# moss-lab/ScanFold

Measured on AMD Instinct MI355X. Metric: windows/sec (W=120, step=1, 100 shuffles), higher is better.
Workload: dtype int32 (int16 LDS storage) energies; f64 partition function

## Files before the change

scanfold_amd/csrc/sf_mfe_fast.hip.h:

```cpp
#pragma once
#include <type_traits>
#include "sf_energy.h"
#include "sf_pk16.h"

#define SF_FAST_NR 34
#ifndef SF_FAST_TINY_D0
#define SF_FAST_TINY_D0 10
#endif
#define SF_FAST_CHUNK_D0 36
#ifndef SF_FAST_UNPACK
#define SF_FAST_UNPACK 1
#endif
#ifndef SF_UNP_PB
#define SF_UNP_PB 4
#endif
#define SF_HELP_MERGE_MAXW 118
#define SF_DML_HELPER_BIAS_256 26
#define SF_DML_HELPER_BIAS_W200 50
#define SF_DML_HELPER_BIAS(ng, wt) ((ng) == 256 ? ((wt) == 200 ? SF_DML_HELPER_BIAS_W200 : SF_DML_HELPER_BIAS_256) : 100000)
#define SF_HELP_NB_128 4
#define SF_HELP_NB_128G 8
#define SF_HELP_NB_256 6
#define SF_INF16 30000
#define SF_FAST_THRESH 10000
// ... 219 lines not shown
      b[k] = pbl[BP ? k * S : (NB - 1 - k) * (S - 1)];
    }
    SF_SPLIT_REDUCE()
  } else {
#pragma unroll
    for (int k = 0; k < NB; k++) {
      const int t = k < NB - 1 ? sfd_min(k, len - 1) : len - 1;
      a[k] = pa[t * sa];
      b[k] = pb[t * sb];
    }
    SF_SPLIT_REDUCE()
  }
#undef SF_SPLIT_REDUCE
}

__device__ __forceinline__ void sf_fast_publish_bn(int16_t *w, const int i0, const uint32_t bn) {
  w[0] = (int16_t)sf_lo(bn);
  if (i0 > 0) w[-1] = (int16_t)sf_hi(bn);
}

#ifdef SF_EMUL
#define SF_GATHER16(F, field, idx) ((int)(F)->field[idx])
#else
__device__ __forceinline__ int sf_gather16_at(const void *base, unsigned off) {
  asm("" : "+v"(off));
  return *(const int16_t *)((const char *)base + (size_t)off);
}
#define SF_GATHER16(F, field, idx) \
  (FOLD ? sf_gather16_at((F), (unsigned)offsetof(SfFastParams, field) + ((unsigned)(idx) << 1)) : (int)(F)->field[idx])
#endif

#ifdef SF_EMUL
static thread_local const char *sf_emul_bn_base = nullptr, *sf_emul_ci_base = nullptr;
static inline void sf_emul_check_bn_row(const char *row_ptr, long lane_bytes, long row_bytes, bool fold) {
  if (!sf_emul_bn_base) return;
  const long row = (row_ptr - sf_emul_bn_base - lane_bytes) / row_bytes;
  if (row < 0 || row > (fold ? SF_FAST_NR - 1 : SF_FAST_NR)) {
    fprintf(stderr, "sf_mfe_fast (emulation): bulge / 1xn row %ld outside the ring and its mirror row\n", row);
    abort();
  }
}
static inline void sf_emul_check_ci_row(const int16_t *row_ptr, long lane_entries, long row_entries, bool fold) {
  if (!sf_emul_ci_base) return;
  const long row = ((const char *)row_ptr - sf_emul_ci_base - 2 * lane_entries) / (2 * row_entries);
  if (row < 0 || row > (fold ? SF_FAST_NR - 1 : SF_FAST_NR)) {
    fprintf(stderr, "sf_mfe_fast (emulation): generic-loop row %ld outside the ring and its mirror row\n", row);
    abort();
  }
}
#endif

enum { SF_SEC_P1 = 1, SF_SEC_HELP = 2, SF_SEC_DML = 4, SF_SEC_FIN = 8, SF_SEC_C0 = 16, SF_SEC_ALL = 31, SF_SEC_PRE = 32,
       SF_SEC_POST = 64 };
struct SfHU {
  short v[27];
};
struct SfPub {
  uint32_t a;
  uint32_t b;
  int tau;
  int type;
};
template <bool G, int WT, int SEC, bool CH = false, bool FOLD = false, int UCAP = SFD_MAXLOOP, int TBLK = 1, bool MGH = false,
          bool UNP = false>
__device__ __forceinline__ void sf_fast_cell(const SfFastCtx &X, const int d, const int i, const bool valid,
                                             const int slot2, const int slotd, uint32_t (&HP)[14], SfHU &HU, int &ovf,
                                             const bool final_fml, const int fnb, int &fpart, int &dec, int &eh, int &e0,
                                             int &dprev, SfPub &pub, const int dml_lo = SFD_TURN + 1,
                                             const int dml_hi = 1 << 20) {
  const SfFastParams *const Fc = FOLD ? X.F : sf_const_base(X.F);
  const int16_t *const ubase = G ? X.uNIN : (CH ? Fc->uniG[sfd_max(sfd_min(d - 2 - (SFD_TURN + 1), 30), 0)] : Fc->uni);
  const int16_t *const uNIN = ubase, *const uIL = ubase + 32, *const uBN = ubase + 64;
#define CBAT(x) X.BN[2 * (x)]
#define C1NAT(x) X.BN[2 * ((x) - 1) + 1]
#define HGET(x) (((x)&1) ? ((int)HP[(x) >> 1] >> 16) : (int)(int16_t)(HP[(x) >> 1] & 0xffffu))
#define HSET(x, v)                                                                                       \
  HP[(x) >> 1] = ((x)&1) ? ((HP[(x) >> 1] & 0x0000ffffu) | ((uint32_t)(v) << 16))                         \
                         : ((HP[(x) >> 1] & 0xffff0000u) | ((uint32_t)(v)&0xffffu))
  const int W = WT ? WT : X.W, RW = W - 4;
// ... 15 lines not shown
    const int tau_in = tr > 2 ? X.TAU : 0;
    int stem, ext;
    if (i > 1 && j < W) { stem = X.tM[SF_TIDX(type, sp1, sq1)]; ext = X.tE[SF_TIDX(type, sp1, sq1)]; }
    else if (i > 1) stem = ext = X.tD5[type * 5 + sp1];
    else if (j < W) stem = ext = X.tD3[type * 5 + sq1];
    else stem = ext = 0;
    pub.a = sf_pk(X.tI[SF_TIDX(tr, sq1, sp1)], X.t1n[SF_TIDX(tr, sq1, sp1)]);
    pub.b = sf_pk(stem + tau_in + X.MLintern, ext + tau_in);
    pub.tau = tau_in;
  }
#define FBASE(dd) (FOLD ? ((dd) <= (W + 3) / 2 ? ((dd)-4) * (W - 3) : (W - 1 - (dd)) * (W - 3) + (dd)-3) \
                        : (((dd)-4) * W - ((dd) * ((dd)-1) / 2 - 6) + (((dd)-4 + (W & 1)) >> 1)))
#define FLEN(dd) (W - (dd) + ((W - (dd)) & 1))
#define ROW(u) ((slot2 - (u) < 0 ? slot2 - (u) + SF_FAST_NR : slot2 - (u)) * RW)
  constexpr bool TBL = !G && TBLK != 0;
  const SfFastRows *const Rc = TBL ? sf_const_base(X.R) : X.R;
  const int32_t *const rci_o = Rc->ci_odd[slot2], *const rci_e = Rc->ci_even[slot2];
  const int32_t *const rbn_o = Rc->bn_odd[slot2], *const rbn_e = Rc->bn_even[slot2];
#define ROWB_CI(u) (TBL ? (((u)&1) ? rci_o[(u) >> 1] : rci_e[(u) >> 1]) : 2 * ROW(u))
#define ROWB_BN(u) (TBL ? (((u)&1) ? rbn_o[(u) >> 1] : rbn_e[(u) >> 1]) : 4 * ROW(u))
#define CIROW(u) ((const int16_t *)((const char *)X.CI + ROWB_CI(u)))

  if (SEC & SF_SEC_P1) {
  if (UNP) {
    static_assert(!UNP || (!G && !CH && !FOLD), "the unpacked recurrence exists for the all-sizes code of the narrow kernel only");
    const int32_t *const nin = Fc->NIN;
    short r30a = 0, r30b = 0;
    {
      const int16_t *row = CIROW(30) + i0;
      r30a = row[3]; r30b = row[29];
    }
    constexpr int PB = SF_UNP_PB;
#pragma unroll
    for (int pb = 12; pb >= 1; pb -= PB) {
      short a3[PB], au[PB], b3[PB], bu[PB];
#pragma unroll
      for (int k = 0; k < PB; k++) {
        if (pb - k >= 1) {
          const int u = 2 * (pb - k) + 4;
          const int16_t *rb = CIROW(u + 1) + i0, *ra = rb + RW;
#ifdef SF_EMUL
          sf_emul_check_ci_row(ra, i0, RW, FOLD); sf_emul_check_ci_row(rb, i0, RW, FOLD);
#endif
          a3[k] = ra[3]; au[k] = ra[u - 1];
          b3[k] = rb[3]; bu[k] = rb[u];
        }
      }
      if (pb == 12) {
        const short e = (short)(sf_opaque16(sfd_min16(r30a, r30b)) + (short)nin[26]);
        HU.v[26] = sf_opaque16(sfd_min16(e, HU.v[24]));
      }
#pragma unroll
      for (int k = 0; k < PB; k++) {
        if (pb - k >= 1) {
          const int x = 2 * (pb - k);
          const short ea = (short)(sf_opaque16(sfd_min16(a3[k], au[k])) + (short)nin[x]);
          const short eb = (short)(sf_opaque16(sfd_min16(b3[k], bu[k])) + (short)nin[x + 1]);
          HU.v[x + 1] = sf_opaque16(sfd_min16(eb, HU.v[x - 1]));
          HU.v[x] = sf_opaque16(sfd_min16(ea, HU.v[x - 2]));
        }
      }
    }
    {
      const int16_t *row = CIROW(5) + i0;
      HU.v[1] = (short)(sfd_min16((short)row[3], (short)row[4]) + (short)nin[1]);
      HU.v[0] = (short)((short)(CIROW(4) + i0)[3] + (short)nin[0]);
    }
  } else {
  if (G) {
#pragma unroll
    for (int u = 30; u >= 6; --u) {
      if (u <= UCAP && u <= umax) {
        const int16_t *row = X.CI + ROW(u) + i0;
        const int e = sfd_min(row[3], row[u - 1]) + SF_UNI(uNIN, u - 4);
        HSET(u - 4, sfd_min(e, HGET(u - 6)));
      }
    }
  } else {
    if (!CH || um >= 30) {
// ... 71 lines not shown
      }
      if (!G || (UCAP >= 3 && umax >= 3)) {
        const int16_t *row = BNROWB(ROWB_BN(3));
        const unsigned ta = RP[S[i + 2] * 8 + S[j - 3]];
        eh = sfd_min(eh, row[2 * 2] + SF_GATHER16(Fc, int21a, (((tq + ta) * 5u + si1) * 5u + S[j - 2]) * 5u + sj1));
        const unsigned tb = RP[S[i + 3] * 8 + S[j - 2]];
        eh = sfd_min(eh, row[2 * 3] + SF_GATHER16(Fc, int21b, (((tb * 8u + type) * 5u + sj1) * 5u + si1) * 5u + S[i + 2]));
      }
      if (!G || (UCAP >= 4 && umax >= 4)) {
        const unsigned t2r = RP[S[i + 3] * 8 + S[j - 3]];
        eh = sfd_min(eh, BNROWB(ROWB_BN(4))[2 * 3] +
                             SF_GATHER16(Fc, int22T, ((((tq + t2r) * 5u + si1) * 5u + S[i + 2]) * 5u + S[j - 2]) * 5u + sj1));
      }
      if (!G || (UCAP >= 5 && umax >= 5)) {
        const int16_t *row = BNROWB(ROWB_BN(5));
        const int m23 = X.t23[SF_TIDX(type, si1, sj1)] + Fc->L23;
        const int ta = RP[S[i + 3] * 8 + S[j - 4]];
        eh = sfd_min(eh, row[2 * 3] + m23 + X.t23in[SF_TIDX(ta, S[j - 3], S[i + 2])]);
        const int tb = RP[S[i + 4] * 8 + S[j - 3]];
        eh = sfd_min(eh, row[2 * 4] + m23 + X.t23in[SF_TIDX(tb, S[j - 2], S[i + 3])]);
      }
      int gb = SF_FAST_BIG, g1 = SF_FAST_BIG;
      if (G) {
#pragma unroll
        for (int u = 2; u <= 30; ++u) {
          if (u <= UCAP && u <= umax) {
            const int rw = ROW(u) + i0;
            gb = sfd_min(gb, sfd_min(CBAT(rw + 1), CBAT(rw + 1 + u)) + SF_UNI(uBN, 2 * u));
            if (u >= 4) g1 = sfd_min(g1, sfd_min(C1NAT(rw + 2), C1NAT(rw + u)) + SF_UNI(uBN, 2 * u + 1));
          }
        }
      } else {
        constexpr bool STAGED = (WT == 120);
        uint32_t acc = sf_pk(32767, 32767), accb = acc;
        constexpr int SF_HELP_NB = FOLD ? SF_HELP_NB_256 : (TBLK == 2 ? SF_HELP_NB_128G : SF_HELP_NB_128);
#pragma unroll
        for (int ub = 2; ub <= 30; ub += SF_HELP_NB) {
          if (CH && ub > um) continue;
          uint32_t w0[SF_HELP_NB], w2[SF_HELP_NB], w3[SF_HELP_NB], wt[SF_HELP_NB], t[SF_HELP_NB];
#pragma unroll
          for (int k = 0; k < SF_HELP_NB; k++) {
            const int u = ub + k;
            if (u <= 30) {
              const int16_t *tp = (FOLD || MGH || u == 30) ? BNROWB(ROWB_BN(u)) : BNROWB(ROWB_BN(u | 1)) + ((u & 1) ? 0 : 2 * RW);
#ifdef SF_EMUL
              sf_emul_check_bn_row((const char *)tp, 4 * i0, 4 * RW, FOLD);
#endif
              w0[k] = sf_ldw(tp + 2 * 1);
              w2[k] = sf_ldw(tp + 2 * (u - 1)); w3[k] = sf_ldw(tp + 2 * (u + 1));
              wt[k] = sf_ldw(uBN + 2 * u);
            }
          }
          if (STAGED) {
#pragma unroll
            for (int k = 0; k < SF_HELP_NB; k++) {
              const int u = ub + k;
              if (u <= 30) {
                const uint32_t x = w0[k];
                const uint32_t y = (w3[k] & 0xffffu) | (w2[k] & 0xffff0000u);
                t[k] = sf_pkmin(x, y);
              }
            }
            SF_VALU_FENCE();
#pragma unroll
            for (int k = 0; k < SF_HELP_NB; k++)
              if (ub + k <= 30) t[k] = sf_pkadd(t[k], wt[k]);
            SF_VALU_FENCE();
#pragma unroll
            for (int k = 0; k + 1 < SF_HELP_NB; k += 2)
              if (ub + k + 1 <= 30) t[k] = sf_pkmin(t[k], t[k + 1]);
            SF_VALU_FENCE();
#pragma unroll
            for (int k = 0; k < SF_HELP_NB; k += 2)
              if (ub + k <= 30) { if (k & 2) accb = sf_pkmin(accb, t[k]); else acc = sf_pkmin(acc, t[k]); }
          } else {
#pragma unroll
            for (int k = 0; k < SF_HELP_NB; k++) {
              const int u = ub + k;
              if (u <= 30) {
                const uint32_t x = w0[k];
                const uint32_t y = (w3[k] & 0xffffu) | (w2[k] & 0xffff0000u);
                acc = sf_pkmin(acc, sf_pkadd(sf_pkmin(x, y), wt[k]));
              }
            }
          }
        }
        acc = sf_pkmin(acc, accb);
        gb = sf_lo(acc); g1 = sf_hi(acc);
      }
      eh = sfd_min(eh, gb + tau_out);
      eh = sfd_min(eh, g1 + X.t1n[SF_TIDX(type, si1, sj1)]);
    }
  }

// ... 68 lines not shown
          const int n = size == 4 ? X.D->P.n_tetra : (size == 6 ? X.D->P.n_hexa : X.D->P.n_tri);
          const uint32_t key = sfd_loop_key(S, i, size + 2);
          for (int k0 = ((n + 7) & ~7) - 8; k0 >= 0; k0 -= 8) {
#pragma unroll
            for (int k = 7; k >= 0; --k) e = keys[k0 + k] == key ? (int)en[k0 + k] : e;
          }
        }
      } else e = X.D->hp_init[d - 1] + X.tH[SF_TIDX(type, si1, sj1)];
      if (!G || umax >= 0) {
        int gg = SF_FAST_BIG;
        if (UNP) {
          const int32_t *const il = Fc->IL;
          short g0 = (short)(HU.v[2] + (short)il[6]), g1 = (short)(HU.v[3] + (short)il[7]);
#pragma unroll
          for (int x = 4; x <= 26; x += 2) {
            g0 = sfd_min16(g0, sf_opaque16((short)(HU.v[x] + (short)il[x + 4])));
            if (x + 1 <= 26) g1 = sfd_min16(g1, sf_opaque16((short)(HU.v[x + 1] + (short)il[x + 5])));
          }
          gg = sfd_min16(g0, g1);
        } else if (G) {
#pragma unroll
          for (int u = 6; u <= 30; ++u)
            if (u <= UCAP && u <= umax) gg = sfd_min(gg, HGET(u - 4) + SF_UNI(uIL, u));
        } else {
          uint32_t ggp = sf_pk(32767, 32767);
#pragma unroll
          for (int pp = 1; pp <= 13; pp++)
            if (!CH || um >= 2 * pp + 4) ggp = sf_pkmin(ggp, sf_pkadd(HP[pp], sf_ldw(uIL + 2 * pp + 4)));
          gg = sfd_min(sf_lo(ggp), sf_hi(ggp));
        }
        e = sfd_min(e, gg + X.tI[SF_TIDX(type, si1, sj1)]);
      }
// ... 33 lines not shown
    const uint32_t bn = sf_pk(c + tau_in, c + X.t1n[SF_TIDX(tr, sq1, sp1)]);
    sf_fast_publish_bn(X.BN + 2 * rbd, i0, bn);
    if (X.bn_dup && slotd == 0) sf_fast_publish_bn(X.BN + 2 * (SF_FAST_NR * RW + i0), i0, bn);
    int stem, ext;
    if (i > 1 && j < W) { stem = X.tM[SF_TIDX(type, sp1, sq1)]; ext = X.tE[SF_TIDX(type, sp1, sq1)]; }
    else if (i > 1) stem = ext = X.tD5[type * 5 + sp1];
    else if (j < W) stem = ext = X.tD3[type * 5 + sq1];
    else stem = ext = 0;
    f = c + stem + tau_in + X.MLintern;
    cx = sfd_min(c + ext + tau_in, SF_INF16);
  } else {
    X.CI[rbd] = SF_INF16; sf_fast_publish_bn(X.BN + 2 * rbd, i0, sf_pk(SF_INF16, SF_INF16));
    if (!FOLD && slotd == 0) X.CI[SF_FAST_NR * RW + i0] = SF_INF16;
    if (X.bn_dup && slotd == 0) sf_fast_publish_bn(X.BN + 2 * (SF_FAST_NR * RW + i0), i0, sf_pk(SF_INF16, SF_INF16));
  }
  X.cg[SF_CGIDX(i, j)] = (int16_t)cx;
  if (final_fml && d > SFD_TURN + 1) f = sfd_min(f, fnb);
  if ((SEC & SF_SEC_DML) && (SEC & SF_SEC_FIN)) multiloop_split();
  f = sfd_min(f, dec);
  dprev = dec > SF_FAST_THRESH ? SF_INF16 : dec;
  fpart = f;
  if (final_fml && f < SF_FAST_OVF) ovf = 1;
  X.fML[FBASE(d) + i0] = (int16_t)(f > SF_FAST_THRESH ? SF_INF16 : f);
#undef ROW
#undef ROWB_CI
#undef ROWB_BN
#undef CIROW
#undef BNROWB
}

// ... 359 lines not shown
                                                int32_t *__restrict__ out, int *__restrict__ ovf_cnt,
                                                int *__restrict__ ovf_list) {
  if (lane == 0) {
    out[seq] = T.f3n;
    if (over || T.f3n < SF_FAST_OVF) {
      const int k = atomicAdd(ovf_cnt, 1);
      ovf_list[k] = seq;
    }
  }
}


enum SfStep {
  SF_STEP_SIZED,
  SF_STEP_GUARDED,
  SF_STEP_UNSPLIT,
  SF_STEP_SPLIT,
  SF_STEP_SPLIT16,
  SF_STEP_SPLIT8,
  SF_STEP_NARROW,
};
template <SfStep K>
using SfStepTag = std::integral_constant<SfStep, K>;
enum SfRole {
  SF_ROLE_ALL,
  SF_ROLE_MAIN_EVEN,
  SF_ROLE_MAIN_ODD,
  SF_ROLE_HELP_EVEN,
  SF_ROLE_HELP_ODD,
};
// ... 21 lines not shown
  const int W = WT ? WT : Wrt;
  SF_DYN_SMEM(smem);
  const SfFastLayout Lo = sf_fast_layout(W, HC);
  SfFastCtx X;
  char *const hcC = (char *)(smem + Lo.off_hc);
  uint8_t *const hcP = (uint8_t *)hcC + (W + 2), *const hcE = hcP + (W + 2);
  int16_t *const scS = (int16_t *)(smem + Lo.off_hc + (((3 * (W + 2)) + 1) & ~1));
  X.hc.c = (HC && cons_rows) ? hcC : nullptr; X.hc.partner = hcP; X.hc.encl = hcE;
  X.sc = (HC && sc_rows) ? scS : nullptr;
  X.fML = (int16_t *)smem;
  X.CI = (int16_t *)(smem + Lo.off_ci);
  X.C1N = nullptr; X.CB = nullptr;
  X.BN = (int16_t *)(smem + Lo.off_c1n);
#ifdef SF_EMUL
  sf_emul_bn_base = (const char *)X.BN; sf_emul_ci_base = (const char *)X.CI;
#endif
  X.DMLr = nullptr;
  int16_t *tab = (int16_t *)(smem + Lo.off_tab);
  X.t23 = tab; X.tI = tab + 175 - 25; X.t1n = tab + 325 - 25; X.tM = tab + 475 - 25; X.tH = tab + 625 - 25;
  X.tE = tab + 775 - 25; X.cg_ext = 1;
  X.tStack = tab + 925; X.tD5 = tab + 989; X.tD3 = tab + 1029;
  uint8_t *tPair = (uint8_t *)(tab + 1069);
  X.tPair = tPair;
  uint8_t *tRPair = (uint8_t *)(tab + SF_FAST_TAB_OLD);
  int16_t *t23in = tab + SF_FAST_TAB_OLD + 32;
  X.tRPair = tRPair; X.t23in = t23in;
  int32_t *flag = (int32_t *)(smem + Lo.off_flag);
  uint8_t *S = (uint8_t *)(smem + Lo.off_S);
  X.S = S;
  X.D = D; X.F = F; X.R = Rows; X.W = W; X.fold = FOLD; X.maxd = D->max_pair_dist;
  constexpr bool MERGE = MG && (NG == 128);
  constexpr bool UNPK = SF_FAST_UNPACK && (NG == 128);
  constexpr bool LGLOOPS = MG && (NG == 128);
  constexpr bool ROLE_LOOPS = (NG == 128);
  constexpr int TBLK = WT > 0 ? 1 : (NG == 128 ? (MG ? 2 : 1) : 0);
  X.bn_dup = (NG == 128);
  uint8_t *const cell_list = (MG && W >= SF_HELP_MERGE_MAXW) ? (uint8_t *)((int16_t *)(smem + Lo.off_tab) + 1069 + 32 + 1)
                                                            : (uint8_t *)(smem + Lo.off_list);
  X.TAU = D->P.TerminalAU; X.MLbase = D->P.MLbase; X.MLclosing = D->P.MLclosing; X.MLintern = D->P.MLintern[1];
  int32_t *f5s = (int32_t *)(smem + Lo.off_ci);
  int16_t *tExt = (int16_t *)(smem + Lo.off_ci + (((W + 1) * 4 + 3) & ~3));

  const int tid = threadIdx.x;
  X.cg = cg_all + (size_t)sf_fast_scratch_slot(blockIdx.x, gridDim.x) * SF_CG_ENTRIES(W);
  for (int x = tid; x < 175; x += NT) {
    tab[x] = F->mm23[x];
    if (x < 150) {
// ... 32 lines not shown
  const int defer_need = n_split_steps > 0 ? (W - SFD_TURN - 1 + n_split_steps - 1) / n_split_steps : 0;
  const int defer_rows = sfd_min(defer_need, DROWS);
  const bool defer_on = n_split_steps >= 8 && defer_need <= 4;
  SfTrail<NQ> T;
#pragma unroll
  for (int q = 0; q < NQ; q++) T.F[q] = 0;
  T.f3n = 0; T.row = 0;

  int *const next_slot = (int *)(smem + Lo.off_next);
  int seq = blockIdx.x;
  while (seq < n) {
    const uint8_t *src = seqs + (size_t)seq * W;
    constexpr bool PINF = true;
    int tidf = tid;
    if (PINF) SF_PIN(tidf);
    __syncthreads();
    if (PZ) {
      for (int x = tid; x < Lo.off_tab / 2; x += NT) ((int16_t *)smem)[x] = sf_poison16(poison, x);
      if (HC) for (int x = tid; x < (Lo.total - Lo.off_hc) / 2; x += NT) ((int16_t *)(smem + Lo.off_hc))[x] = sf_poison16(poison, x);
      __syncthreads();
    }
    for (int x = tidf; x < W; x += NT) S[x + 1] = sf_encode_nt(src[x]);
    if (MG && W >= SF_HELP_MERGE_MAXW) for (int x = tidf; x < 128; x += NT) ((int16_t *)(smem + Lo.off_tab) + 1069 + 32 + 1)[x] = F->uni[x];
    for (int x = tidf; x < (Lo.off_tab - Lo.off_ci) / 4; x += NT) ((uint32_t *)X.CI)[x] = sf_pk(SF_INF16, SF_INF16);
    int fetched = 0;
    if (tid == 0) {
      S[0] = 0; S[W + 1] = 0; flag[0] = 0;
      fetched = (int)gridDim.x + atomicAdd(work_ctr, 1);
    }
    __syncthreads();
    if (HC) {
      if (cons_rows)
        for (int x = tid; x < W; x += NT) hcC[x + 1] = cons_rows[(size_t)seq * W + x];
      if (sc_rows)
        for (int x = tid; x < W; x += NT) scS[x + 1] = (int16_t)sfd_max(sfd_min(sc_rows[(size_t)seq * W + x], 30000), -30000);
      __syncthreads();
      if (cons_rows && tid == 0) flag[0] = sf_hc_parse8(W, hcC, hcP, hcE) ? 2 : 0;
      __syncthreads();
      if (cons_rows && flag[0] == 2) {
// ... 20 lines not shown
    int slot2 = (SFD_TURN + 1 + grp - 2) % SF_FAST_NR, slotd = (SFD_TURN + 1 + grp) % SF_FAST_NR;
    auto build_list = [&](const int dd0) {
      const int lane = tid & 63;
      const int d1 = dd0 + 1;
      const int iH = ((v - 64) & (NG - 1)) - (dd0 >> 1);
      const bool vA = (dd0 < W) && (iH >= 1) && (iH + dd0 <= W), vB = (d1 < W) && (iH >= 1) && (iH + d1 <= W);
      const int tA = (vA && dd0 <= X.maxd) ? X.tPair[S[iH] * 8 + S[iH + dd0]] : 0;
      const int tB = (vB && d1 <= X.maxd) ? X.tPair[S[iH] * 8 + S[iH + d1]] : 0;
      const unsigned long long mA = __ballot(tA != 0), mB = __ballot(tB != 0);
      const int cA = __popcll(mA);
      uint8_t *list = cell_list + (((dd0 >> 1) & 1) << 7);
      const unsigned long long below = (1ull << lane) - 1ull;
      if (tA) list[__popcll(mA & below)] = (uint8_t)iH;
      if (tB) list[cA + __popcll(mB & below)] = (uint8_t)(iH | 128);
      if (lane == 0) list[127] = (uint8_t)(cA + __popcll(mB));
    };
    SfHU HU;
    const int grp_wave = grp;
    const bool sweeper_wave = sweeper;
    auto step = [&](const int d0, auto kind_tag, auto role_tag) {
      constexpr SfStep KIND = decltype(kind_tag)::value;
      constexpr SfRole ROLE = decltype(role_tag)::value;
      constexpr bool ROLES = ROLE != SF_ROLE_ALL;
      static_assert(!ROLES || (NG == 128 && KIND >= SF_STEP_SPLIT && KIND <= SF_STEP_SPLIT8), "roles: the narrow kernel's split steps");
      const int grp = ROLES ? (int)(ROLE == SF_ROLE_MAIN_ODD || ROLE == SF_ROLE_HELP_ODD) : grp_wave;
      const bool hwave = ROLES ? ROLE >= SF_ROLE_HELP_EVEN : tg >= 64;
      const bool sweeper = ROLES ? ROLE == SF_ROLE_HELP_ODD : sweeper_wave;
      constexpr int LGC = KIND == SF_STEP_SPLIT16 ? 4 : (KIND == SF_STEP_SPLIT8 ? 3 : (KIND == SF_STEP_SPLIT && LGLOOPS ? 5 : 0));
      constexpr bool DO_G = KIND == SF_STEP_SIZED, DO_CH = KIND == SF_STEP_GUARDED;
      const int d = d0 + grp;
      if (!ROLES && d0 == SFD_TURN + 1 + 2 && tid == 0) *next_slot = fetched;
      if (!ROLES && d0 == SFD_TURN + 1 + 4) next_seq = SF_WAVE_UNIFORM(*next_slot);
      constexpr bool split = KIND >= SF_STEP_SPLIT;
      constexpr bool narrow = KIND == SF_STEP_NARROW;
      if (NARROW && d0 == narrow_d0) {
        uint32_t *const xa = (uint32_t *)X.BN;
        const int RWc = W - 4;
        if (tg >= 96 && tg < 160) {
#pragma unroll
          for (int k = 0; k < 14; k++) xa[(grp * 16 + k) * RWc + 100 + (tg - 96)] = H[k];
          xa[(grp * 16 + 14) * RWc + 100 + (tg - 96)] = (uint32_t)dprev;
          xa[(grp * 16 + 15) * RWc + 100 + (tg - 96)] = (uint32_t)fnb;
        }
        __syncthreads();
        if (tg >= 64 && tg < 128) {
// ... 19 lines not shown
      int dec = SF_FAST_BIG, eh = SF_FAST_BIG, e0 = SF_FAST_BIG;
      SfPub pub;
      pub.a = pub.b = 0; pub.tau = 0; pub.type = 0;
      int dc[DROWS][NQ];
      const bool sweep_now = defer_on && sweeper && split && T.row > 0;
      const int sweep_rows = sweep_now ? sfd_max(sfd_min(defer_rows, T.row - (W - d0)), 0) : 0;
      if (sweep_now) {
#pragma unroll
        for (int k = 0; k < DROWS; k++)
          if (k < sweep_rows) sf_trail_load<NQ>(X.cg, W, tid & 63, T.row - k, dc[k]);
      }
      if (__ballot(valid)) {
        if (DO_G && d0 < 8) sf_fast_cell<true, WT, SF_SEC_ALL, false, FOLD, 1>(X, d, i, valid, slot2, slotd, H, HU, ovf, grp == 0, fnb, fpart, dec, eh, e0, dprev, pub);
        else if (DO_G && d0 < SF_FAST_TINY_D0) sf_fast_cell<true, WT, SF_SEC_ALL, false, FOLD, 5>(X, d, i, valid, slot2, slotd, H, HU, ovf, grp == 0, fnb, fpart, dec, eh, e0, dprev, pub);
        else if (DO_CH && d0 < SF_FAST_CHUNK_D0) sf_fast_cell<false, WT, SF_SEC_ALL, true, FOLD, SFD_MAXLOOP, TBLK>(X, d, i, valid, slot2, slotd, H, HU, ovf, grp == 0, fnb, fpart, dec, eh, e0, dprev, pub);
        else if (!split) sf_fast_cell<false, WT, SF_SEC_ALL, false, FOLD, SFD_MAXLOOP, TBLK, false, UNPK && KIND == SF_STEP_UNSPLIT>(X, d, i, valid, slot2, slotd, H, HU, ovf, grp == 0, fnb, fpart, dec, eh, e0, dprev, pub);
        else if (DML4 && narrow) {
          const int nmain = dml_terms / 5, cA = SFD_TURN + 1 + nmain, cB = cA + (dml_terms - nmain + 1) / 2;
          uint32_t *const xa = (uint32_t *)X.BN;
          if (dmlw) {
            const bool wB = tg >= 192;
            sf_fast_cell<false, WT, SF_SEC_DML, false, FOLD, SFD_MAXLOOP, TBLK>(X, d, i, valid, slot2, slotd, H, HU, ovf, false, fnb, fpart, dec, eh, e0, dprev, pub, wB ? cB : cA, wB ? (1 << 20) : cB - 1);
            if (valid) xa[(grp * 16 + (wB ? 1 : 0)) * (W - 4) + 100 + (tg & 63)] = (uint32_t)sfd_min(dec, 32000);
          } else if (!helper) {
            sf_fast_cell<false, WT, SF_SEC_P1 | SF_SEC_C0 | SF_SEC_DML | SF_SEC_PRE, false, FOLD, SFD_MAXLOOP, TBLK>(X, d, i, valid, slot2, slotd, H, HU, ovf, grp == 0, fnb, fpart, dec, eh, e0, dprev, pub, SFD_TURN + 1, cA - 1);
          } else {
            sf_fast_cell<false, WT, SF_SEC_HELP, false, FOLD, SFD_MAXLOOP, TBLK>(X, d, i, valid, slot2, slotd, H, HU, ovf, grp == 0, fnb, fpart, dec, eh, e0, dprev, pub);
            if (valid) X.BN[2 * (slotd * (W - 4) + i - 1)] = (int16_t)sfd_min(eh, 32000);
          }
        }
// ... 7 lines not shown
        } else if (MERGE) {
          const int lane = tid & 63;
          const uint8_t *list = cell_list + (((d0 >> 1) & 1) << 7);
          const int cT = SF_WAVE_UNIFORM((int)list[127]);
          const int e = (grp << 6) + lane;
          if (SF_WAVE_UNIFORM(cT > (grp << 6))) {
            const bool vC = e < cT;
            const int ent = vC ? list[e] : 1;
            const int g = ent >> 7, iC = ent & 127;
            const int s2 = slot2 - grp < 0 ? slot2 - grp + SF_FAST_NR : slot2 - grp;
            const int sd0 = slotd - grp < 0 ? slotd - grp + SF_FAST_NR : slotd - grp;
            const int sd1 = sd0 + 1 >= SF_FAST_NR ? 0 : sd0 + 1;
            SfFastCtx Xh = X;
            Xh.BN = X.BN + 2 * g * (W - 4);
            sf_fast_cell<false, WT, SF_SEC_HELP, false, FOLD, SFD_MAXLOOP, TBLK, true>(Xh, d0 + g, iC, vC, s2, sd0, H, HU, ovf, false, fnb, fpart, dec, eh, e0, dprev, pub);
            if (vC) X.BN[2 * ((g ? sd1 : sd0) * (W - 4) + iC - 1)] = (int16_t)sfd_min(eh, 32000);
          }
        } else {
          if (SHARE) {
            sf_fast_cell<false, WT, SF_SEC_HELP | SF_SEC_DML, false, FOLD, SFD_MAXLOOP, TBLK>(X, d, i, valid, slot2, slotd, H, HU, ovf, grp == 0, fnb, fpart, dec, eh, e0, dprev, pub, dml_cut);
            if (valid) {
              X.BN[2 * (slotd * (W - 4) + i - 1)] = (int16_t)sfd_min(eh, 32000);
              X.CI[slotd * (W - 4) + i - 1] = (int16_t)sfd_min(dec, 32000);
            }
          } else {
            sf_fast_cell<false, WT, SF_SEC_HELP, false, FOLD, SFD_MAXLOOP, TBLK>(X, d, i, valid, slot2, slotd, H, HU, ovf, grp == 0, fnb, fpart, dec, eh, e0, dprev, pub);
            if (valid) X.BN[2 * (slotd * (W - 4) + i - 1)] = (int16_t)sfd_min(eh, 32000);
          }
        }
      }
      if (sweep_now && sweep_rows > 0) sf_trail_rows<NQ, DROWS>(T, tid & 63, sweep_rows, dc);
      if (MERGE && grp == 1 && hwave && (ROLES || d0 + 2 >= split_d0) && d0 + 2 < W) build_list(d0 + 2);
      if (split) {
        __syncthreads();
        if (!helper && !dmlw && __ballot(valid)) {
          if (valid) {
            eh = X.BN[2 * (slotd * (W - 4) + i - 1)];
            if (DML4 && narrow) {
              const uint32_t *const xa = (const uint32_t *)X.BN;
              dec = sfd_min(dec, sfd_min((int)xa[(grp * 16) * (W - 4) + 100 + (tg & 63)], (int)xa[(grp * 16 + 1) * (W - 4) + 100 + (tg & 63)]));
            } else if (SHARE) dec = sfd_min(dec, (int)X.CI[slotd * (W - 4) + i - 1]);
          }
// ... 7 lines not shown
        const bool ex0 = i + d1 <= W, ex1 = i >= 2;
        const int ia = i - 1, ib = ex1 ? i - 2 : 0;
        const int p0 = pd[ia], p1 = pd[ib], q0 = pe[i], q1 = pe[ia], q2 = pe[ib];
        const int v0 = sfd_min(p0, sfd_min(q0, q1) + X.MLbase), v1 = sfd_min(p1, sfd_min(q1, q2) + X.MLbase);
        if ((ex0 && v0 < SF_FAST_OVF) || (ex1 && v1 < SF_FAST_OVF)) ovf = 1;
        const int g0 = (ex0 && v0 <= SF_FAST_THRESH) ? v0 : SF_INF16, g1 = (ex1 && v1 <= SF_FAST_THRESH) ? v1 : SF_INF16;
        if (ex0) X.fML[FBASE(d1) + ia] = (int16_t)g0;
        fnb = sfd_min(g0, g1) + X.MLbase;
      }
      slot2 += 2; if (slot2 >= SF_FAST_NR) slot2 -= SF_FAST_NR;
      slotd += 2; if (slotd >= SF_FAST_NR) slotd -= SF_FAST_NR;
    };
    {
      int d0 = SFD_TURN + 1;
      constexpr SfRoleTag<SF_ROLE_ALL> all_roles{};
      for (; d0 < SF_FAST_TINY_D0 && d0 < W; d0 += 2) step(d0, SfStepTag<SF_STEP_SIZED>{}, all_roles);
      for (; d0 < SF_FAST_CHUNK_D0 && d0 < W; d0 += 2) step(d0, SfStepTag<SF_STEP_GUARDED>{}, all_roles);
      if constexpr (UNPK) {
#pragma unroll
        for (int x = 0; x < 27; x++) HU.v[x] = (short)((x & 1) ? (H[x >> 1] >> 16) : (H[x >> 1] & 0xffffu));
      }
      for (; d0 < split_d0 && d0 < W; d0 += 2) step(d0, SfStepTag<SF_STEP_UNSPLIT>{}, all_roles);
      auto split_loops = [&](auto role_tag) {
        if constexpr (LGLOOPS) {
          for (; d0 < W - 30 && d0 < W; d0 += 2) step(d0, SfStepTag<SF_STEP_SPLIT>{}, role_tag);
          for (; d0 < W - 14 && d0 < W; d0 += 2) step(d0, SfStepTag<SF_STEP_SPLIT16>{}, role_tag);
          for (; d0 < W; d0 += 2) step(d0, SfStepTag<SF_STEP_SPLIT8>{}, role_tag);
        }
        for (; d0 < W; d0 += 2) step(d0, SfStepTag<SF_STEP_SPLIT>{}, role_tag);
      };
      if constexpr (ROLE_LOOPS) {
        const int wave = SF_WAVE_UNIFORM(tid >> 6);
        if (wave == 0) split_loops(SfRoleTag<SF_ROLE_MAIN_EVEN>{});
        else if (wave == 2) split_loops(SfRoleTag<SF_ROLE_MAIN_ODD>{});
        else if (wave == 1) split_loops(SfRoleTag<SF_ROLE_HELP_EVEN>{});
// ... 101 lines not shown
```

Before: 46090.

## Add capped-loop-size step variants for short diagonals using unpacked recurrence

Result: faster. 47170 (median of 6 runs) (+2.4%).

```diff
diff --git a/scanfold_amd/csrc/sf_mfe_fast.hip.h b/scanfold_amd/csrc/sf_mfe_fast.hip.h
--- a/scanfold_amd/csrc/sf_mfe_fast.hip.h
+++ b/scanfold_amd/csrc/sf_mfe_fast.hip.h
@@ -1,5 +1,8 @@
 #pragma once
 #include <type_traits>
+#ifdef SF_EMUL
+#include <vector>
+#endif
 #include "sf_energy.h"
 #include "sf_pk16.h"
 
@@ -8,6 +11,16 @@
 #define SF_FAST_TINY_D0 10
 #endif
 #define SF_FAST_CHUNK_D0 36
+#ifndef SF_FAST_SHORT
+#define SF_FAST_SHORT 1
+#endif
+#ifndef SF_FAST_SHORT_D1
+#define SF_FAST_SHORT_D1 18
+#endif
+#ifndef SF_FAST_SHORT_D2
+#define SF_FAST_SHORT_D2 26
+#endif
+#define SF_FAST_SHORT_D3 32
 #ifndef SF_FAST_UNPACK
 #define SF_FAST_UNPACK 1
 #endif
@@ -257,11 +270,6 @@
 #undef SF_SPLIT_REDUCE
 }
 
-__device__ __forceinline__ void sf_fast_publish_bn(int16_t *w, const int i0, const uint32_t bn) {
-  w[0] = (int16_t)sf_lo(bn);
-  if (i0 > 0) w[-1] = (int16_t)sf_hi(bn);
-}
-
 #ifdef SF_EMUL
 #define SF_GATHER16(F, field, idx) ((int)(F)->field[idx])
 #else
@@ -291,7 +299,64 @@
     abort();
   }
 }
-#endif
+static thread_local std::vector<unsigned char> sf_emul_shadow;
+static thread_local const char *sf_emul_span_lo = nullptr, *sf_emul_span_hi = nullptr;
+static inline void sf_emul_shadow_span(const char *lo, const char *hi) {
+  sf_emul_span_lo = lo; sf_emul_span_hi = hi;
+  if (sf_emul_shadow.size() != (size_t)(hi - lo) / 2) sf_emul_shadow.assign((size_t)(hi - lo) / 2, 2);
+}
+static inline void sf_emul_shadow_set(const void *p, int n16, unsigned char v) {
+  const char *q = (const char *)p;
+  if (!sf_emul_span_lo || q < sf_emul_span_lo || q + 2 * n16 > sf_emul_span_hi) return;
+  for (int k = 0; k < n16; k++) sf_emul_shadow[(size_t)(q - sf_emul_span_lo) / 2 + k] = v;
+}
+static inline void sf_emul_check_absent(const void *p, int n16, int d, int u) {
+  const char *q = (const char *)p;
+  if (!sf_emul_span_lo) return;
+  if (q < sf_emul_span_lo || q + 2 * n16 > sf_emul_span_hi) {
+    fprintf(stderr, "sf_mfe_fast (emulation): read for loop size %d, absent on diagonal %d, outside the rolling tables and their mirror rows (%ld bytes past their end)\n",
+            u, d, (long)(q + 2 * n16 - sf_emul_span_hi));
+    abort();
+  }
+  for (int k = 0; k < n16; k++) {
+    const int s = sf_emul_shadow[(size_t)(q - sf_emul_span_lo) / 2 + k];
+    if (s != 0) {
+      fprintf(stderr, "sf_mfe_fast (emulation): read for loop size %d, absent on diagonal %d, finds an entry %s (entry %ld of the rolling tables)\n",
+              u, d, s == 1 ? "a diagonal of this fold has written" : "this fold's prologue has not initialised", (long)((q - sf_emul_span_lo) / 2 + k));
+      abort();
+    }
+  }
+}
+extern "C" int sfemul_absent_check_selftest(int W, int what) {
+  const SfFastLayout L = sf_fast_layout(W);
+  static std::vector<char> lds;
+  lds.assign((size_t)L.total, 0);
+  sf_emul_shadow_span(lds.data() + L.off_ci, lds.data() + L.off_tab);
+  sf_emul_shadow_set(lds.data() + L.off_ci, (L.off_tab - L.off_ci) / 2, 0);
+  if (what == 0) {
+    const int16_t *e = (const int16_t *)(lds.data() + L.off_ci) + 3 * (W - 4) + 3;
+    sf_emul_check_absent(e, 1, 10, 5);
+    sf_emul_shadow_set(e, 1, 1);
+    sf_emul_check_absent(e, 1, 10, 5);
+  } else {
+    sf_emul_check_absent(lds.data() + L.off_tab - 4, 2, 10, 8);
+    sf_emul_check_absent(lds.data() + L.off_tab, 2, 10, 8);
+  }
+  return 0;
+}
+#define SF_EMUL_WROTE(p, n16) sf_emul_shadow_set((p), (n16), 1)
+#define SF_EMUL_ABSENT(CHK, p, n16, d, u) do { if ((CHK) && (u) > (d) - 2 - (SFD_TURN + 1)) sf_emul_check_absent((p), (n16), (d), (u)); } while (0)
+#else
+#define SF_EMUL_WROTE(p, n16) ((void)0)
+#define SF_EMUL_ABSENT(CHK, p, n16, d, u) ((void)0)
+#endif
+
+__device__ __forceinline__ void sf_fast_publish_bn(int16_t *w, const int i0, const uint32_t bn) {
+  w[0] = (int16_t)sf_lo(bn);
+  if (i0 > 0) w[-1] = (int16_t)sf_hi(bn);
+  SF_EMUL_WROTE(w, 1);
+  if (i0 > 0) SF_EMUL_WROTE(w - 1, 1);
+}
 
 enum { SF_SEC_P1 = 1, SF_SEC_HELP = 2, SF_SEC_DML = 4, SF_SEC_FIN = 8, SF_SEC_C0 = 16, SF_SEC_ALL = 31, SF_SEC_PRE = 32,
        SF_SEC_POST = 64 };
@@ -305,7 +370,7 @@
   int type;
 };
 template <bool G, int WT, int SEC, bool CH = false, bool FOLD = false, int UCAP = SFD_MAXLOOP, int TBLK = 1, bool MGH = false,
-          bool UNP = false>
+          bool UNP = false, bool SHORT = false>
 __device__ __forceinline__ void sf_fast_cell(const SfFastCtx &X, const int d, const int i, const bool valid,
                                              const int slot2, const int slotd, uint32_t (&HP)[14], SfHU &HU, int &ovf,
                                              const bool final_fml, const int fnb, int &fpart, int &dec, int &eh, int &e0,
@@ -351,6 +416,8 @@
 #define FLEN(dd) (W - (dd) + ((W - (dd)) & 1))
 #define ROW(u) ((slot2 - (u) < 0 ? slot2 - (u) + SF_FAST_NR : slot2 - (u)) * RW)
   constexpr bool TBL = !G && TBLK != 0;
+  constexpr int UTOP = (!G && UCAP < SFD_MAXLOOP) ? UCAP : SFD_MAXLOOP;
+  constexpr bool UNG = !G && !CH;
   const SfFastRows *const Rc = TBL ? sf_const_base(X.R) : X.R;
   const int32_t *const rci_o = Rc->ci_odd[slot2], *const rci_e = Rc->ci_even[slot2];
   const int32_t *const rbn_o = Rc->bn_odd[slot2], *const rbn_e = Rc->bn_even[slot2];
@@ -362,9 +429,11 @@
   if (UNP) {
     static_assert(!UNP || (!G && !CH && !FOLD), "the unpacked recurrence exists for the all-sizes code of the narrow kernel only");
     const int32_t *const nin = Fc->NIN;
+    static_assert(!UNP || UTOP >= 7, "the unpacked recurrence keeps at least the sizes 6 and 7");
     short r30a = 0, r30b = 0;
-    {
+    if (UTOP >= 30) {
       const int16_t *row = CIROW(30) + i0;
+      SF_EMUL_ABSENT(true, row + 3, 1, d, 30); SF_EMUL_ABSENT(true, row + 29, 1, d, 30);
       r30a = row[3]; r30b = row[29];
     }
     constexpr int PB = SF_UNP_PB;
@@ -373,23 +442,25 @@
       short a3[PB], au[PB], b3[PB], bu[PB];
 #pragma unroll
       for (int k = 0; k < PB; k++) {
-        if (pb - k >= 1) {
+        if (pb - k >= 1 && 2 * (pb - k) + 4 <= UTOP) {
           const int u = 2 * (pb - k) + 4;
           const int16_t *rb = CIROW(u + 1) + i0, *ra = rb + RW;
 #ifdef SF_EMUL
           sf_emul_check_ci_row(ra, i0, RW, FOLD); sf_emul_check_ci_row(rb, i0, RW, FOLD);
 #endif
+          SF_EMUL_ABSENT(true, ra + 3, 1, d, u); SF_EMUL_ABSENT(true, ra + u - 1, 1, d, u);
+          SF_EMUL_ABSENT(true, rb + 3, 1, d, u + 1); SF_EMUL_ABSENT(true, rb + u, 1, d, u + 1);
           a3[k] = ra[3]; au[k] = ra[u - 1];
           b3[k] = rb[3]; bu[k] = rb[u];
         }
       }
-      if (pb == 12) {
+      if (pb == 12 && UTOP >= 30) {
         const short e = (short)(sf_opaque16(sfd_min16(r30a, r30b)) + (short)nin[26]);
         HU.v[26] = sf_opaque16(sfd_min16(e, HU.v[24]));
       }
 #pragma unroll
       for (int k = 0; k < PB; k++) {
-        if (pb - k >= 1) {
+        if (pb - k >= 1 && 2 * (pb - k) + 4 <= UTOP) {
           const int x = 2 * (pb - k);
           const short ea = (short)(sf_opaque16(sfd_min16(a3[k], au[k])) + (short)nin[x]);
           const short eb = (short)(sf_opaque16(sfd_min16(b3[k], bu[k])) + (short)nin[x + 1]);
@@ -400,6 +471,7 @@
     }
     {
       const int16_t *row = CIROW(5) + i0;
+      SF_EMUL_ABSENT(true, row + 3, 2, d, 5); SF_EMUL_ABSENT(true, CIROW(4) + i0 + 3, 1, d, 4);
       HU.v[1] = (short)(sfd_min16((short)row[3], (short)row[4]) + (short)nin[1]);
       HU.v[0] = (short)((short)(CIROW(4) + i0)[3] + (short)nin[0]);
     }
@@ -501,7 +573,8 @@
       }
       if (!G || (UCAP >= 5 && umax >= 5)) {
         const int16_t *row = BNROWB(ROWB_BN(5));
-        const int m23 = X.t23[SF_TIDX(type, si1, sj1)] + Fc->L23;
+        SF_EMUL_ABSENT(UNG, row + 2 * 3, 1, d, 5); SF_EMUL_ABSENT(UNG, row + 2 * 4, 1, d, 5);
+        const int m23= X.t23[SF_TIDX(type, si1, sj1)] + Fc->L23;
         const int ta = RP[S[i + 3] * 8 + S[j - 4]];
         eh = sfd_min(eh, row[2 * 3] + m23 + X.t23in[SF_TIDX(ta, S[j - 3], S[i + 2])]);
         const int tb = RP[S[i + 4] * 8 + S[j - 3]];
@@ -522,17 +595,18 @@
         uint32_t acc = sf_pk(32767, 32767), accb = acc;
         constexpr int SF_HELP_NB = FOLD ? SF_HELP_NB_256 : (TBLK == 2 ? SF_HELP_NB_128G : SF_HELP_NB_128);
 #pragma unroll
-        for (int ub = 2; ub <= 30; ub += SF_HELP_NB) {
+        for (int ub = 2; ub <= UTOP; ub += SF_HELP_NB) {
           if (CH && ub > um) continue;
           uint32_t w0[SF_HELP_NB], w2[SF_HELP_NB], w3[SF_HELP_NB], wt[SF_HELP_NB], t[SF_HELP_NB];
 #pragma unroll
           for (int k = 0; k < SF_HELP_NB; k++) {
             const int u = ub + k;
-            if (u <= 30) {
-              const int16_t *tp = (FOLD || MGH || u == 30) ? BNROWB(ROWB_BN(u)) : BNROWB(ROWB_BN(u | 1)) + ((u & 1) ? 0 : 2 * RW);
+            if (u <= UTOP) {
+              const int16_t *tp = (FOLD || MGH || SHORT || u == 30) ? BNROWB(ROWB_BN(u)) : BNROWB(ROWB_BN(u | 1)) + ((u & 1) ? 0 : 2 * RW);
 #ifdef SF_EMUL
               sf_emul_check_bn_row((const char *)tp, 4 * i0, 4 * RW, FOLD);
 #endif
+              SF_EMUL_ABSENT(UNG, tp + 2 * 1, 2, d, u); SF_EMUL_ABSENT(UNG, tp + 2 * (u - 1), 2, d, u); SF_EMUL_ABSENT(UNG, tp + 2 * (u + 1), 2, d, u);
               w0[k] = sf_ldw(tp + 2 * 1);
               w2[k] = sf_ldw(tp + 2 * (u - 1)); w3[k] = sf_ldw(tp + 2 * (u + 1));
               wt[k] = sf_ldw(uBN + 2 * u);
@@ -542,7 +616,7 @@
 #pragma unroll
             for (int k = 0; k < SF_HELP_NB; k++) {
               const int u = ub + k;
-              if (u <= 30) {
+              if (u <= UTOP) {
                 const uint32_t x = w0[k];
                 const uint32_t y = (w3[k] & 0xffffu) | (w2[k] & 0xffff0000u);
                 t[k] = sf_pkmin(x, y);
@@ -551,20 +625,20 @@
             SF_VALU_FENCE();
 #pragma unroll
             for (int k = 0; k < SF_HELP_NB; k++)
-              if (ub + k <= 30) t[k] = sf_pkadd(t[k], wt[k]);
+              if (ub + k <= UTOP) t[k] = sf_pkadd(t[k], wt[k]);
             SF_VALU_FENCE();
 #pragma unroll
             for (int k = 0; k + 1 < SF_HELP_NB; k += 2)
-              if (ub + k + 1 <= 30) t[k] = sf_pkmin(t[k], t[k + 1]);
+              if (ub + k + 1 <= UTOP) t[k] = sf_pkmin(t[k], t[k + 1]);
             SF_VALU_FENCE();
 #pragma unroll
             for (int k = 0; k < SF_HELP_NB; k += 2)
-              if (ub + k <= 30) { if (k & 2) accb = sf_pkmin(accb, t[k]); else acc = sf_pkmin(acc, t[k]); }
+              if (ub + k <= UTOP) { if (k & 2) accb = sf_pkmin(accb, t[k]); else acc = sf_pkmin(acc, t[k]); }
           } else {
 #pragma unroll
             for (int k = 0; k < SF_HELP_NB; k++) {
               const int u = ub + k;
-              if (u <= 30) {
+              if (u <= UTOP) {
                 const uint32_t x = w0[k];
                 const uint32_t y = (w3[k] & 0xffffu) | (w2[k] & 0xffff0000u);
                 acc = sf_pkmin(acc, sf_pkadd(sf_pkmin(x, y), wt[k]));
@@ -663,8 +737,8 @@
           short g0 = (short)(HU.v[2] + (short)il[6]), g1 = (short)(HU.v[3] + (short)il[7]);
 #pragma unroll
           for (int x = 4; x <= 26; x += 2) {
-            g0 = sfd_min16(g0, sf_opaque16((short)(HU.v[x] + (short)il[x + 4])));
-            if (x + 1 <= 26) g1 = sfd_min16(g1, sf_opaque16((short)(HU.v[x + 1] + (short)il[x + 5])));
+            if (x + 4 <= UTOP) g0 = sfd_min16(g0, sf_opaque16((short)(HU.v[x] + (short)il[x + 4])));
+            if (x + 1 <= 26 && x + 5 <= UTOP) g1 = sfd_min16(g1, sf_opaque16((short)(HU.v[x + 1] + (short)il[x + 5])));
           }
           gg = sfd_min16(g0, g1);
         } else if (G) {
@@ -728,6 +802,8 @@
     if (!FOLD && slotd == 0) X.CI[SF_FAST_NR * RW + i0] = SF_INF16;
     if (X.bn_dup && slotd == 0) sf_fast_publish_bn(X.BN + 2 * (SF_FAST_NR * RW + i0), i0, sf_pk(SF_INF16, SF_INF16));
   }
+  SF_EMUL_WROTE(X.CI + rbd, 1);
+  if (!FOLD && slotd == 0) SF_EMUL_WROTE(X.CI + SF_FAST_NR * RW + i0, 1);
   X.cg[SF_CGIDX(i, j)] = (int16_t)cx;
   if (final_fml && d > SFD_TURN + 1) f = sfd_min(f, fnb);
   if ((SEC & SF_SEC_DML) && (SEC & SF_SEC_FIN)) multiloop_split();
@@ -1117,6 +1193,9 @@
 enum SfStep {
   SF_STEP_SIZED,
   SF_STEP_GUARDED,
+  SF_STEP_SHORT_A,
+  SF_STEP_SHORT_B,
+  SF_STEP_SHORT_C,
   SF_STEP_UNSPLIT,
   SF_STEP_SPLIT,
   SF_STEP_SPLIT16,
@@ -1168,6 +1247,7 @@
   X.BN = (int16_t *)(smem + Lo.off_c1n);
 #ifdef SF_EMUL
   sf_emul_bn_base = (const char *)X.BN; sf_emul_ci_base = (const char *)X.CI;
+  sf_emul_shadow_span((const char *)(smem + Lo.off_ci), (const char *)(smem + Lo.off_tab));
 #endif
   X.DMLr = nullptr;
   int16_t *tab = (int16_t *)(smem + Lo.off_tab);
@@ -1185,6 +1265,9 @@
   X.D = D; X.F = F; X.R = Rows; X.W = W; X.fold = FOLD; X.maxd = D->max_pair_dist;
   constexpr bool MERGE = MG && (NG == 128);
   constexpr bool UNPK = SF_FAST_UNPACK && (NG == 128);
+  constexpr bool SHORTU = SF_FAST_SHORT && UNPK && !HC;
+  static_assert(SF_FAST_TINY_D0 >= 10 && SF_FAST_TINY_D0 <= SF_FAST_SHORT_D1 && SF_FAST_SHORT_D1 <= SF_FAST_SHORT_D2 &&
+                SF_FAST_SHORT_D2 <= SF_FAST_SHORT_D3 && SF_FAST_SHORT_D1 >= 14, "SHORT loops: d0 >= 10 (no tabulated hairpin, sizes 0 .. 4 exist), caps >= 7");
   constexpr bool LGLOOPS = MG && (NG == 128);
   constexpr bool ROLE_LOOPS = (NG == 128);
   constexpr int TBLK = WT > 0 ? 1 : (NG == 128 ? (MG ? 2 : 1) : 0);
@@ -1247,6 +1330,9 @@
     constexpr bool PINF = true;
     int tidf = tid;
     if (PINF) SF_PIN(tidf);
+#ifdef SF_EMUL
+    if (tid == 0) sf_emul_shadow_set(smem + Lo.off_ci, (Lo.off_tab - Lo.off_ci) / 2, 2);
+#endif
     __syncthreads();
     if (PZ) {
       for (int x = tid; x < Lo.off_tab / 2; x += NT) ((int16_t *)smem)[x] = sf_poison16(poison, x);
@@ -1255,7 +1341,12 @@
     }
     for (int x = tidf; x < W; x += NT) S[x + 1] = sf_encode_nt(src[x]);
     if (MG && W >= SF_HELP_MERGE_MAXW) for (int x = tidf; x < 128; x += NT) ((int16_t *)(smem + Lo.off_tab) + 1069 + 32 + 1)[x] = F->uni[x];
-    for (int x = tidf; x < (Lo.off_tab - Lo.off_ci) / 4; x += NT) ((uint32_t *)X.CI)[x] = sf_pk(SF_INF16, SF_INF16);
+    for (int x = tidf; x < (Lo.off_tab - Lo.off_ci) / 4; x += NT) {
+      ((uint32_t *)X.CI)[x] = sf_pk(SF_INF16, SF_INF16);
+#ifdef SF_EMUL
+      sf_emul_shadow_set((uint32_t *)X.CI + x, 2, 0);
+#endif
+    }
     int fetched = 0;
     if (tid == 0) {
       S[0] = 0; S[W + 1] = 0; flag[0] = 0;
@@ -1306,6 +1397,7 @@
       if (tA) list[__popcll(mA & below)] = (uint8_t)iH;
       if (tB) list[cA + __popcll(mB & below)] = (uint8_t)(iH | 128);
       if (lane == 0) list[127] = (uint8_t)(cA + __popcll(mB));
+      if (lane == 0) SF_EMUL_WROTE(list, 64);
     };
     SfHU HU;
     const int grp_wave = grp;
@@ -1321,6 +1413,8 @@
       constexpr int LGC = KIND == SF_STEP_SPLIT16 ? 4 : (KIND == SF_STEP_SPLIT8 ? 3 : (KIND == SF_STEP_SPLIT && LGLOOPS ? 5 : 0));
       constexpr bool DO_G = KIND == SF_STEP_SIZED, DO_CH = KIND == SF_STEP_GUARDED;
       const int d = d0 + grp;
+      constexpr bool DO_SH = KIND >= SF_STEP_SHORT_A && KIND <= SF_STEP_SHORT_C;
+      constexpr int SHCAP = KIND == SF_STEP_SHORT_A ? SF_FAST_SHORT_D1 - 7 : (KIND == SF_STEP_SHORT_B ? SF_FAST_SHORT_D2 - 7 : SFD_MAXLOOP);
       if (!ROLES && d0 == SFD_TURN + 1 + 2 && tid == 0) *next_slot = fetched;
       if (!ROLES && d0 == SFD_TURN + 1 + 4) next_seq = SF_WAVE_UNIFORM(*next_slot);
       constexpr bool split = KIND >= SF_STEP_SPLIT;
@@ -1370,6 +1464,7 @@
         if (DO_G && d0 < 8) sf_fast_cell<true, WT, SF_SEC_ALL, false, FOLD, 1>(X, d, i, valid, slot2, slotd, H, HU, ovf, grp == 0, fnb, fpart, dec, eh, e0, dprev, pub);
         else if (DO_G && d0 < SF_FAST_TINY_D0) sf_fast_cell<true, WT, SF_SEC_ALL, false, FOLD, 5>(X, d, i, valid, slot2, slotd, H, HU, ovf, grp == 0, fnb, fpart, dec, eh, e0, dprev, pub);
         else if (DO_CH && d0 < SF_FAST_CHUNK_D0) sf_fast_cell<false, WT, SF_SEC_ALL, true, FOLD, SFD_MAXLOOP, TBLK>(X, d, i, valid, slot2, slotd, H, HU, ovf, grp == 0, fnb, fpart, dec, eh, e0, dprev, pub);
+        else if (DO_SH) sf_fast_cell<false, WT, SF_SEC_ALL, false, FOLD, SHORTU ? SHCAP : SFD_MAXLOOP, TBLK, false, SHORTU, SHORTU>(X, d, i, valid, slot2, slotd, H, HU, ovf, grp == 0, fnb, fpart, dec, eh, e0, dprev, pub);
         else if (!split) sf_fast_cell<false, WT, SF_SEC_ALL, false, FOLD, SFD_MAXLOOP, TBLK, false, UNPK && KIND == SF_STEP_UNSPLIT>(X, d, i, valid, slot2, slotd, H, HU, ovf, grp == 0, fnb, fpart, dec, eh, e0, dprev, pub);
         else if (DML4 && narrow) {
           const int nmain = dml_terms / 5, cA = SFD_TURN + 1 + nmain, cB = cA + (dml_terms - nmain + 1) / 2;
@@ -1407,7 +1502,7 @@
             SfFastCtx Xh = X;
             Xh.BN = X.BN + 2 * g * (W - 4);
             sf_fast_cell<false, WT, SF_SEC_HELP, false, FOLD, SFD_MAXLOOP, TBLK, true>(Xh, d0 + g, iC, vC, s2, sd0, H, HU, ovf, false, fnb, fpart, dec, eh, e0, dprev, pub);
-            if (vC) X.BN[2 * ((g ? sd1 : sd0) * (W - 4) + iC - 1)] = (int16_t)sfd_min(eh, 32000);
+            if (vC) { X.BN[2 * ((g ? sd1 : sd0) * (W - 4) + iC - 1)] = (int16_t)sfd_min(eh, 32000); SF_EMUL_WROTE(X.BN + 2 * ((g ? sd1 : sd0) * (W - 4) + iC - 1), 1); }
           }
         } else {
           if (SHARE) {
@@ -1418,7 +1513,7 @@
             }
           } else {
             sf_fast_cell<false, WT, SF_SEC_HELP, false, FOLD, SFD_MAXLOOP, TBLK>(X, d, i, valid, slot2, slotd, H, HU, ovf, grp == 0, fnb, fpart, dec, eh, e0, dprev, pub);
-            if (valid) X.BN[2 * (slotd * (W - 4) + i - 1)] = (int16_t)sfd_min(eh, 32000);
+            if (valid) { X.BN[2 * (slotd * (W - 4) + i - 1)] = (int16_t)sfd_min(eh, 32000); SF_EMUL_WROTE(X.BN + 2 * (slotd * (W - 4) + i - 1), 1); }
           }
         }
       }
@@ -1456,11 +1551,19 @@
     {
       int d0 = SFD_TURN + 1;
       constexpr SfRoleTag<SF_ROLE_ALL> all_roles{};
+      auto unpack_state = [&]() {
+#pragma unroll
+        for (int x = 0; x < 27; x++) HU.v[x] = (short)((x & 1) ? (H[x >> 1] >> 16) : (H[x >> 1] & 0xffffu));
+      };
       for (; d0 < SF_FAST_TINY_D0 && d0 < W; d0 += 2) step(d0, SfStepTag<SF_STEP_SIZED>{}, all_roles);
-      for (; d0 < SF_FAST_CHUNK_D0 && d0 < W; d0 += 2) step(d0, SfStepTag<SF_STEP_GUARDED>{}, all_roles);
-      if constexpr (UNPK) {
-#pragma unroll
-        for (int x = 0; x < 27; x++) HU.v[x] = (short)((x & 1) ? (H[x >> 1] >> 16) : (H[x >> 1] & 0xffffu));
+      if constexpr (SHORTU) {
+        unpack_state();
+        for (; d0 < SF_FAST_SHORT_D1 && d0 < W; d0 += 2) step(d0, SfStepTag<SF_STEP_SHORT_A>{}, all_roles);
+        for (; d0 < SF_FAST_SHORT_D2 && d0 < W; d0 += 2) step(d0, SfStepTag<SF_STEP_SHORT_B>{}, all_roles);
+        for (; d0 < SF_FAST_SHORT_D3 && d0 < W; d0 += 2) step(d0, SfStepTag<SF_STEP_SHORT_C>{}, all_roles);
+      } else {
+        for (; d0 < SF_FAST_CHUNK_D0 && d0 < W; d0 += 2) step(d0, SfStepTag<SF_STEP_GUARDED>{}, all_roles);
+        if constexpr (UNPK) unpack_state();
       }
       for (; d0 < split_d0 && d0 < W; d0 += 2) step(d0, SfStepTag<SF_STEP_UNSPLIT>{}, all_roles);
       auto split_loops = [&](auto role_tag) {
```
